# CompVis/behavior-driven-video-synthesis

Hardware: AMD Instinct MI355X
Metric: frames/sec VUnet 256x256 bs=16 fwd+bwd (higher is better)
Workload: dtype f32 (operands scaled by a power of two and split into 2 fp16 terms, 3 partial products on fp16 MFMA, fp32 accumulate; weight gradients and uncovered layers: 3 bf16 terms / 6 products, fp32-input MFMA, fp32 VALU); 1 GPU; Human3.6m shape_and_pose_net VunetAlter 256x256 per-GPU bs=16 fwd+bwd, VGG19 perceptual + KL loss, fused Adam, dropout 0.05, regressor side loop off, seeded-synthetic VGG19 weights, rasterised synthetic stickmen; global_batch=16, parallelism=dp1, conv_precision=h2, hip_streams=4, hip_graph=True, graph_settle_steps=7, rccl_world_size=1, dp_backend=none

## Files before the change

### behavior_driven_video_synthesis_amd/csrc/conv_p2.hip

```cpp
#include <stdio.h>

#include <type_traits>

#include "common.h"
#include "split_h2.h"

namespace {

constexpr int P2_META = 128, P2_AMAX0 = 16, P2_NSLOT = 64;

struct P2Args {
  const uint4* x;
  const int* xmeta;
  const uint4* w;
  const float* wk;
  const float* shift;
  const uint4* mask;
  uint4* y;
  int* ymeta;
  int N, C, H, W, M;
  int relu;
};

__device__ __forceinline__ void p2_dma(uint32_t voff, const void* sbase, uint32_t lds_addr) {
  uint32_t keep;
  asm volatile("s_mov_b32 %0, m0\n\ts_mov_b32 m0, %3\n\ts_nop 0\n\tglobal_load_lds_dwordx4 %1, %2\n\ts_mov_b32 m0, %0"
               : "=&s"(keep)
               : "v"(voff), "s"(sbase), "s"(lds_addr)
               : "memory");
}
template <int N>
__device__ __forceinline__ void p2_dma_wait() {
  static_assert(N == 0 || N == 1 || N == 2 || N == 4, "counts in use");
  if constexpr (N == 0) asm volatile("s_waitcnt vmcnt(0)" ::: "memory");
  else if constexpr (N == 1) asm volatile("s_waitcnt vmcnt(1)" ::: "memory");
  else if constexpr (N == 2) asm volatile("s_waitcnt vmcnt(2)" ::: "memory");
// ... 16 lines not shown

__device__ __forceinline__ void p2_swap16(uint32_t& a, uint32_t& b) {
  const auto r = __builtin_amdgcn_permlane16_swap(a, b, false, false);
  a = r[0];
  b = r[1];
}

__device__ __forceinline__ uint32_t p2_nonzero_halves(uint32_t t) {
  typedef unsigned short u16x2 __attribute__((ext_vector_type(2)));
  u16x2 v = __builtin_bit_cast(u16x2, t);
  const u16x2 one = {1, 1}, all = {0xFFFF, 0xFFFF};
  v = __builtin_elementwise_min(v, one) * all;
  return __builtin_bit_cast(uint32_t, v);
}

#define P2_TERMS 2
#include "conv_p2_kernel.h"
#undef P2_TERMS
#define P2_TERMS 1
#include "conv_p2_kernel.h"
#undef P2_TERMS

template <int CT, int TERMS>
int p2a_launch(const P2Args& a, hipStream_t st) {
  constexpr int XU = 4 * TERMS * 10 * (CT + 2), XS = (XU + 63) / 64 * 64, WU = 128 * 4 * TERMS;
  constexpr size_t lds = (size_t)(2 * XS + 2 * WU) * 16;
  const int blocks = a.N * (a.H / 8) * (a.W / CT) * (a.M / 128);
  void (*kern)(const P2Args);
  if constexpr (TERMS == 2) kern = conv_p2a_kernel<CT>;
  else kern = conv_p2a_kernel<CT, 1>;
  if (hipFuncSetAttribute((const void*)kern, hipFuncAttributeMaxDynamicSharedMemorySize, (int)lds) != hipSuccess) return VUNET_ERR_LAUNCH;
  VUNET_LAUNCH(kern, dim3((unsigned)blocks), dim3(512), lds, st, a);
  return vunet_check_launch();
}

template <int NW, int CT, int XBUF, int TERMS>
int p2_launch(const P2Args& a, hipStream_t st) {
  constexpr int XU = 4 * TERMS * 10 * (CT + 2), XS = (XU + 63) / 64 * 64, WU = 16 * NW * 4 * TERMS;
  constexpr size_t lds = (size_t)(XBUF * XS + 2 * WU) * 16;
  const int blocks = a.N * (a.H / 8) * (a.W / CT) * (a.M / (16 * NW));
  void (*kern)(const P2Args);
  if constexpr (TERMS == 2) kern = conv_p2_kernel<NW, CT, XBUF>;
  else kern = conv_p2_kernel<NW, CT, XBUF, 1>;
  if (lds > 64 * 1024 && hipFuncSetAttribute((const void*)kern, hipFuncAttributeMaxDynamicSharedMemorySize, (int)lds) != hipSuccess)
    return VUNET_ERR_LAUNCH;
  VUNET_LAUNCH(kern, dim3((unsigned)blocks), dim3(64 * NW), lds, st, a);
  return vunet_check_launch();
}

}

static bool p2_shape_ok(const vunet_p2_desc* d) {
  if (!d || d->N < 1 || d->C < 32 || d->C % 32 || d->M < 64 || d->M % 64 || d->H < 8 || d->H % 8) return false;
  if (!(d->W == 16 || (d->W >= 32 && d->W % 32 == 0))) return false;
  const double plane_bytes = (double)d->N * (d->C / 8) * (d->H + 2) * (d->W + 2) * 16.0;
  return plane_bytes * 2.0 < 4.0e9;
}

// ... 11 lines not shown
  int form;
  bool lockstep;
  int xbuf;
};
static P2Route p2_route(const vunet_p2_desc* d, bool dgrad) {
  const int mode = g_vunet_tune[VUNET_TUNE_P2_TERMS], force = g_vunet_tune[VUNET_TUNE_P2_FORM];
  if (mode == 3 && dgrad) {
    if (d->M % 128 == 0 && (force == 2 || force == 3)) return {1, 8, false, 2};
    const long wgs = (long)d->N * (d->H / 8) * (d->W / (d->W == 16 ? 16 : 32)) * (d->M / 64);
    return {1, 4, false, force != 1 && wgs <= 256 ? 2 : 1};
  }
  const int terms = mode == 1 ? 1 : 2, form = p2_form(d);
  return {terms, form, terms == 2 && force == 3, form == 8 ? 2 : 1};
}

extern "C" int vunet_p2_conv(const vunet_p2_desc* d, const void* x, const int32_t* xmeta, const void* w_image, const float* wk,
                             const float* shift, const void* mask, void* y, int32_t* ymeta, void* stream) {
  if (!d || !x || !xmeta || !w_image || !wk || !y || !ymeta) return VUNET_ERR_ARG;
  if (!p2_shape_ok(d)) return VUNET_ERR_UNSUPPORTED;
  if (((uintptr_t)x | (uintptr_t)w_image | (uintptr_t)y | (uintptr_t)mask | (uintptr_t)shift) & 15) return VUNET_ERR_ARG;
  P2Args a;
  a.x = (const uint4*)x; a.xmeta = xmeta; a.w = (const uint4*)w_image; a.wk = wk; a.shift = shift; a.mask = (const uint4*)mask;
  a.y = (uint4*)y; a.ymeta = ymeta;
  a.N = d->N; a.C = d->C; a.H = d->H; a.W = d->W; a.M = d->M; a.relu = d->relu;
  hipStream_t st = (hipStream_t)stream;
  const P2Route r = p2_route(d, d->relu == 0 && shift == nullptr);
  if (r.terms == 2) {
    if (d->W == 16) return r.form == 8 ? (r.lockstep ? p2_launch<8, 16, 2, 2>(a, st) : p2a_launch<16, 2>(a, st)) : p2_launch<4, 16, 1, 2>(a, st);
    return r.form == 8 ? (r.lockstep ? p2_launch<8, 32, 2, 2>(a, st) : p2a_launch<32, 2>(a, st)) : p2_launch<4, 32, 1, 2>(a, st);
  }
  if (r.form == 8 || r.xbuf == 1) {
    if (d->W == 16) return r.form == 8 ? p2a_launch<16, 1>(a, st) : p2_launch<4, 16, 1, 1>(a, st);
    return r.form == 8 ? p2a_launch<32, 1>(a, st) : p2_launch<4, 32, 1, 1>(a, st);
  }
  return d->W == 16 ? p2_launch<4, 16, 2, 1>(a, st) : p2_launch<4, 32, 2, 1>(a, st);
}

extern "C" int vunet_p2_conv_variant(const vunet_p2_desc* d, char* name, int32_t len) {
  if (!d || !name || len < 32) return VUNET_ERR_ARG;
  if (!p2_shape_ok(d)) return VUNET_ERR_UNSUPPORTED;
  const P2Route r = p2_route(d, d->relu == 0);
  const int ct = d->W == 16 ? 16 : 32;
  if (r.terms == 1) {
    if (r.form == 8) snprintf(name, (size_t)len, "conv_p2a_kernel<%d, 1>", ct);
    else snprintf(name, (size_t)len, "conv_p2_kernel<4, %d, %d, 1>", ct, r.xbuf);
    return VUNET_OK;
  }
  if (r.form == 8 && !r.lockstep) snprintf(name, (size_t)len, "conv_p2a_kernel<%d>", ct);
  else snprintf(name, (size_t)len, "conv_p2_kernel<%d, %d, %d>", r.form, ct, r.xbuf);
  return VUNET_OK;
// ... 145 lines not shown
    for (int j = 0; j < 8; ++j) {
      float f = src[j * HW];
      if (relu) f = f > 0.f ? f : 0.f;
      v[j] = f * s;
    }
    uint4 h, l;
    h2_split2(v[0], v[1], h.x, l.x);
    h2_split2(v[2], v[3], h.y, l.y);
    h2_split2(v[4], v[5], h.z, l.z);
    h2_split2(v[6], v[7], h.w, l.w);
    const size_t o = (t * Hp + (yh + 1)) * Wp + (xw + 1);
    y[o] = h;
    y[plane + o] = l;
  }
}
__device__ __forceinline__ void p2_unpack(const uint4& h, const uint4& l, float inv, float* v) {
  const uint32_t hs[4] = {h.x, h.y, h.z, h.w}, ls[4] = {l.x, l.y, l.z, l.w};
#pragma unroll
  for (int j = 0; j < 4; ++j) {
    const h2_f16x2 a = __builtin_bit_cast(h2_f16x2, hs[j]), b = __builtin_bit_cast(h2_f16x2, ls[j]);
    v[2 * j] = ((float)a[0] + (float)b[0] * (1.f / 2048.f)) * inv;
    v[2 * j + 1] = ((float)a[1] + (float)b[1] * (1.f / 2048.f)) * inv;
  }
}
__global__ __launch_bounds__(256) void p2_to_nchw_kernel(const uint4* __restrict__ x, const int* __restrict__ xmeta,
                                                         float* __restrict__ y, int N, int C, int H, int W) {
  const int CB = C >> 3, Hp = H + 2, Wp = W + 2;
  const float inv = h2_pow2(-xmeta[0]);
  const size_t HW = (size_t)H * W, total = (size_t)N * CB * HW, plane = (size_t)N * CB * Hp * Wp;
  for (size_t i = (size_t)blockIdx.x * 256 + threadIdx.x; i < total; i += (size_t)gridDim.x * 256) {
    const int xw = (int)(i % W);
    size_t t = i / W;
    const int yh = (int)(t % H);
    t /= H;
    const size_t o = (t * Hp + (yh + 1)) * Wp + (xw + 1);
    float v[8];
    p2_unpack(x[o], x[plane + o], inv, v);
    float* dst = y + (t * 8) * HW + (size_t)yh * W + xw;
#pragma unroll
// ... 27 lines not shown
```

### behavior_driven_video_synthesis_amd/csrc/conv_p2_kernel.h

```cpp
#if P2_TERMS == 2
template <int NW, int CT, int XBUF>
#else
template <int NW, int CT, int XBUF, int ONE>
#endif
__global__ __launch_bounds__(64 * NW, NW == 8 ? 1 : 2) void conv_p2_kernel(const P2Args a) {
  constexpr int TERMS = P2_TERMS;
  static_assert(NW == 4 || NW == 8, "waves");
  static_assert(CT == 32 || CT == 16, "tile width");
  static_assert(TERMS == 1 || TERMS == 2, "terms per operand");
  constexpr int MW = 16 * NW;
  constexpr int RT = 8, IH = RT + 2, CW = CT + 2, XPIX = IH * CW, XU = 4 * TERMS * XPIX;
  constexpr int NXI = (XU + 63) / 64, XS = NXI * 64;
  constexpr int NXW = (NXI + NW - 1) / NW;
  constexpr int WU = MW * 4 * TERMS;
  constexpr int NWI = WU / 64 / NW;
  constexpr int WSRC = TERMS == 2 ? 1024 : 2048;
  constexpr int PTR = CT / 16, NPT = 2 * PTR;
  static_assert(XBUF == 1 || NXW <= 8, "the next chunk's pieces ride on the first taps");
  extern __shared__ __attribute__((aligned(16))) uint4 smem[];
  uint4* const xL = smem;
  uint4* const wL = smem + XBUF * XS;

  const int tid = threadIdx.x, lane = tid & 63;
  const int wave = __builtin_amdgcn_readfirstlane(tid >> 6);
// ... 43 lines not shown
  };
  auto issue_w = [&](int g, int buf) {
    const char* src = wsrc0 + (size_t)g * wslab;
#pragma unroll
    for (int i = 0; i < NWI; ++i) {
      const int part = wave * NWI + i;
      p2_dma(lane16, p2_uniform_ptr(src + (size_t)part * WSRC), wL_addr + (uint32_t)(buf * WU + part * 64) * 16u);
    }
  };

  issue_w(0, 0);
#pragma unroll
  for (int i = 0; i < NXW; ++i) issue_x(0, i);

  float descale, descale2, sy;
  {
    const int ex = a.xmeta[0];
    const float amax_x = p2_meta_amax(a.xmeta, lane);
    const int ew = (int)a.wk[2];
    h2_pow2_pair(-(ex + ew), descale, descale2);
    const float bound = a.wk[0] * amax_x + a.wk[1];
    const int ey = h2_scale_exp(bound);
    sy = h2_pow2(ey);
    if (blockIdx.x == 0 && tid == 0) a.ymeta[0] = ey;
  }

  f32x4 acc[4][NPT], acx[4][NPT];
#pragma unroll
  for (int mt = 0; mt < 4; ++mt)
#pragma unroll
    for (int q = 0; q < NPT; ++q)
#pragma unroll
      for (int r = 0; r < 4; ++r) acc[mt][q][r] = acx[mt][q][r] = 0.f;

  p2_dma_wait<0>();
  __syncthreads();

// ... 93 lines not shown
      p2_swap16(ll[0][0], ll[1][0]);
      p2_swap16(ll[0][1], ll[1][1]);
      uint4 uh = make_uint4(hh[0][0], hh[0][1], hh[1][0], hh[1][1]);
      uint4 ul = make_uint4(ll[0][0], ll[0][1], ll[1][0], ll[1][1]);
      const int q = qp + (cg & 1);
      const int orow = row0 + 2 * rg + q / PTR, ocol = col0 + (q % PTR) * 16 + px;
      const int cb = ((m0 + 64 * mg + 16 * mt) >> 3) + (cg >> 1);
      const size_t o = (((size_t)n * MB + cb) * Hp + (orow + 1)) * Wp + (ocol + 1);
      if (a.mask) {
        const uint4 mh = a.mask[o], ml = a.mask[plane + o];
        const uint32_t k0 = p2_nonzero_halves((mh.x | ml.x) & 0x7FFF7FFFu), k1 = p2_nonzero_halves((mh.y | ml.y) & 0x7FFF7FFFu);
        const uint32_t k2 = p2_nonzero_halves((mh.z | ml.z) & 0x7FFF7FFFu), k3 = p2_nonzero_halves((mh.w | ml.w) & 0x7FFF7FFFu);
        uh.x &= k0; uh.y &= k1; uh.z &= k2; uh.w &= k3;
        ul.x &= k0; ul.y &= k1; ul.z &= k2; ul.w &= k3;
      }
      a.y[o] = uh;
      a.y[plane + o] = ul;
    }
  }
  {
    const float m_ = wave_max(ymax);
    if (lane == 0)
      atomicMax(reinterpret_cast<unsigned*>(a.ymeta) + P2_AMAX0 + ((blockIdx.x * NW + wave) & (P2_NSLOT - 1)), __float_as_uint(m_));
  }
}

#if P2_TERMS == 2
template <int CT>
#else
template <int CT, int ONE>
#endif
__global__ __launch_bounds__(512, 1) void conv_p2a_kernel(const P2Args a) {
  constexpr int TERMS = P2_TERMS;
  static_assert(TERMS == 1 || TERMS == 2, "terms per operand");
  constexpr int NW = 8, MW = 128;
  constexpr int RT = 8, IH = RT + 2, CW = CT + 2, XPIX = IH * CW, XU = 4 * TERMS * XPIX;
  constexpr int NXI = (XU + 63) / 64, XS = NXI * 64;
  constexpr int NXG = (NXI + 3) / 4;
  constexpr int XPT = 2, NXT = (NXG + XPT - 1) / XPT;
  constexpr int WU = MW * 4 * TERMS;
  constexpr int WSRC = TERMS == 2 ? 1024 : 2048;
  constexpr int PTR = CT / 16, NPT = 2 * PTR;
  static_assert(NXT <= 8, "the next chunk's pieces must be visible before its first tap");
  extern __shared__ __attribute__((aligned(16))) uint4 smem[];
  uint4* const xL = smem;
  uint4* const wL = smem + 2 * XS;

  const int tid = threadIdx.x, lane = tid & 63;
  const int wave = __builtin_amdgcn_readfirstlane(tid >> 6);
  const int mg = wave >> 2, rg = wave & 3;
  const int px = lane & 15, cg = lane >> 4;
  const int Hp = a.H + 2, Wp = a.W + 2, CB = a.C >> 3, MB = a.M >> 3;

  const unsigned bid = xcd_remap(blockIdx.x, gridDim.x);
  const int mblocks = a.M / MW;
  const int mb = bid % mblocks;
  int t = bid / mblocks;
  const int tiles_w = a.W / CT, tiles_h = a.H / RT;
  const int tx = t % tiles_w;
  t /= tiles_w;
  const int ty = t % tiles_h;
  const int n = t / tiles_h;
  const int row0 = ty * RT, col0 = tx * CT, m0 = mb * MW;

  uint32_t xoff[NXG];
#pragma unroll
  for (int i = 0; i < NXG; ++i) {
    int j = rg + 4 * i;
    if (j >= NXI) j = NXI - 1;
    int u = 64 * j + lane;
    if (u >= XU) u = XU - 1;
    const int p = u / (4 * XPIX);
    int rem = u - p * 4 * XPIX;
    const int kq = rem / XPIX;
    rem -= kq * XPIX;
    const int r = rem / CW, c = rem - r * CW;
    xoff[i] = (uint32_t)((((size_t)p * a.N * CB + kq) * Hp + (row0 + r)) * Wp + col0 + c) * 16u;
  }
  const uint32_t xL_addr = (uint32_t)(uintptr_t)(__attribute__((address_space(3))) void*)xL;
  const uint32_t wL_addr = (uint32_t)(uintptr_t)(__attribute__((address_space(3))) void*)wL;
  const char* const xsrc0 = reinterpret_cast<const char*>(a.x) + (size_t)n * CB * Hp * Wp * 16;
  const size_t xchunk = (size_t)4 * Hp * Wp * 16;
  const char* const wsrc0 = reinterpret_cast<const char*>(a.w) + (size_t)mb * (MW / 16) * 128 * 16;
  const size_t wslab = (size_t)(a.M / 16) * 128 * 16;
  const uint32_t lane16 = (uint32_t)lane * 16u;

  auto issue_x = [&](int ch, int i) {
    int j = rg + 4 * i;
    if (j >= NXI) j = NXI - 1;
    if constexpr (TERMS == 1) j = __builtin_amdgcn_readfirstlane(j);
    p2_dma(xoff[i], p2_uniform_ptr(xsrc0 + (size_t)ch * xchunk), xL_addr + (uint32_t)((ch & 1) * XS + 64 * j) * 16u);
  };
  auto issue_w = [&](int g, int buf) {
    const char* src = wsrc0 + (size_t)g * wslab;
#pragma unroll
    for (int i = 0; i < 2 * TERMS; ++i) {
      const int part = rg * (2 * TERMS) + i;
      p2_dma(lane16, p2_uniform_ptr(src + (size_t)part * WSRC), wL_addr + (uint32_t)(buf * WU + part * 64) * 16u);
    }
  };

  if (mg == 0) issue_w(0, 0);
  else {
#pragma unroll
    for (int i = 0; i < NXG; ++i) issue_x(0, i);
  }
  float descale, descale2, sy;
  {
    const int ex = a.xmeta[0];
    const float amax_x = p2_meta_amax(a.xmeta, lane);
    const int ew = (int)a.wk[2];
    h2_pow2_pair(-(ex + ew), descale, descale2);
    const float bound = a.wk[0] * amax_x + a.wk[1];
    const int ey = h2_scale_exp(bound);
    sy = h2_pow2(ey);
    if (blockIdx.x == 0 && tid == 0) a.ymeta[0] = ey;
  }
  f32x4 acc[4][NPT], acx[4][NPT];
#pragma unroll
  for (int mt = 0; mt < 4; ++mt)
#pragma unroll
    for (int q = 0; q < NPT; ++q)
#pragma unroll
      for (int r = 0; r < 4; ++r) acc[mt][q][r] = acx[mt][q][r] = 0.f;
  p2_dma_wait<0>();
  __syncthreads();
  if (mg == 1) __builtin_amdgcn_s_barrier();

  const int nch = a.C >> 5;
  const uint4* const wA0 = wL + (mg * 4) * (64 * TERMS) + lane;
  const uint4* const xB0 = xL + cg * XPIX + px + (2 * rg) * CW;

  auto chunk = [&](int ch, auto last_c) {
    constexpr bool LAST = decltype(last_c)::value;
    const uint4* const xB = xB0 + (ch & 1) * XS;
    const int wpar = (ch * 9) & 1;
#pragma unroll
    for (int tap = 0; tap < 9; ++tap) {
      const int kh = tap / 3, kw = tap - 3 * kh;
      const int g = ch * 9 + tap;
      const int buf = wpar ^ (tap & 1);
      const bool more_w = !(LAST && tap == 8);
      if (mg == 0) {
        if (more_w) issue_w(g + 1, buf ^ 1);
      } else if (!LAST && tap < NXT) {
#pragma unroll
        for (int i = 0; i < XPT; ++i)
          if (tap * XPT + i < NXG) issue_x(ch + 1, tap * XPT + i);
      }
      const uint4* const wA = wA0 + buf * WU;
      P2Unit av[TERMS][4], bv[TERMS][NPT];
#pragma unroll
      for (int p = 0; p < TERMS; ++p) {
#pragma unroll
        for (int mt = 0; mt < 4; ++mt) av[p][mt].u = wA[(mt * TERMS + p) * 64];
#pragma unroll
        for (int q = 0; q < NPT; ++q) bv[p][q].u = xB[p * 4 * XPIX + (q / PTR + kh) * CW + (q % PTR) * 16 + kw];
      }
      asm volatile("s_waitcnt lgkmcnt(0)" ::: "memory");
      __builtin_amdgcn_sched_barrier(0);
      __builtin_amdgcn_s_barrier();
      __builtin_amdgcn_sched_barrier(0);
      __builtin_amdgcn_s_setprio(1);
// ... 9 lines not shown
          for (int q = 0; q < NPT; ++q)
            acx[mt][q] = __builtin_amdgcn_mfma_f32_16x16x32_f16(av[0][mt].b, bv[TERMS - 1][q].b, acx[mt][q], 0, 0, 0);
      }
#pragma unroll
      for (int mt = 0; mt < 4; ++mt)
#pragma unroll
        for (int q = 0; q < NPT; ++q)
          acc[mt][q] = __builtin_amdgcn_mfma_f32_16x16x32_f16(av[0][mt].b, bv[0][q].b, acc[mt][q], 0, 0, 0);
      __builtin_amdgcn_s_setprio(0);
      __builtin_amdgcn_sched_barrier(0);
      p2_dma_wait<0>();
      __builtin_amdgcn_s_barrier();
      __builtin_amdgcn_sched_barrier(0);
    }
  };
  for (int ch = 0; ch + 1 < nch; ++ch) chunk(ch, std::false_type{});
  chunk(nch - 1, std::true_type{});
  if (mg == 0) __builtin_amdgcn_s_barrier();

  const bool relu = a.relu != 0;
  const size_t plane = (size_t)a.N * MB * Hp * Wp;
  float ymax = 0.f;
#pragma unroll
  for (int mt = 0; mt < 4; ++mt) {
    const int co = m0 + 64 * mg + 16 * mt + 4 * cg;
    float sh[4] = {0.f, 0.f, 0.f, 0.f};
    if (a.shift) {
      const float4 s4 = *reinterpret_cast<const float4*>(a.shift + co);
      sh[0] = s4.x; sh[1] = s4.y; sh[2] = s4.z; sh[3] = s4.w;
    }
#pragma unroll
    for (int qp = 0; qp < NPT; qp += 2) {
      uint32_t hh[2][2], ll[2][2];
#pragma unroll
      for (int s = 0; s < 2; ++s) {
        float v[4];
#pragma unroll
        for (int r = 0; r < 4; ++r) {
          float c;
          if constexpr (TERMS == 2) c = (acc[mt][qp + s][r] + acx[mt][qp + s][r] * (1.f / 2048.f)) * descale * descale2 + sh[r];
          else c = acc[mt][qp + s][r] * descale * descale2 + sh[r];
          c = (relu && !(c > 0.f)) ? 0.f : c;
          ymax = fmaxf(ymax, fabsf(c));
          v[r] = c * sy;
        }
        h2_split2(v[0], v[1], hh[s][0], ll[s][0]);
        h2_split2(v[2], v[3], hh[s][1], ll[s][1]);
      }
      p2_swap16(hh[0][0], hh[1][0]);
      p2_swap16(hh[0][1], hh[1][1]);
      p2_swap16(ll[0][0], ll[1][0]);
      p2_swap16(ll[0][1], ll[1][1]);
      uint4 uh = make_uint4(hh[0][0], hh[0][1], hh[1][0], hh[1][1]);
      uint4 ul = make_uint4(ll[0][0], ll[0][1], ll[1][0], ll[1][1]);
      const int q = qp + (cg & 1);
      const int orow = row0 + 2 * rg + q / PTR, ocol = col0 + (q % PTR) * 16 + px;
      const int cb = ((m0 + 64 * mg + 16 * mt) >> 3) + (cg >> 1);
      const size_t o = (((size_t)n * MB + cb) * Hp + (orow + 1)) * Wp + (ocol + 1);
      if (a.mask) {
        const uint4 mh = a.mask[o], ml = a.mask[plane + o];
        const uint32_t k0 = p2_nonzero_halves((mh.x | ml.x) & 0x7FFF7FFFu), k1 = p2_nonzero_halves((mh.y | ml.y) & 0x7FFF7FFFu);
        const uint32_t k2 = p2_nonzero_halves((mh.z | ml.z) & 0x7FFF7FFFu), k3 = p2_nonzero_halves((mh.w | ml.w) & 0x7FFF7FFFu);
        uh.x &= k0; uh.y &= k1; uh.z &= k2; uh.w &= k3;
        ul.x &= k0; ul.y &= k1; ul.z &= k2; ul.w &= k3;
      }
      a.y[o] = uh;
      a.y[plane + o] = ul;
    }
  }
  {
    const float m_ = wave_max(ymax);
    if (lane == 0)
      atomicMax(reinterpret_cast<unsigned*>(a.ymeta) + P2_AMAX0 + ((blockIdx.x * NW + wave) & (P2_NSLOT - 1)), __float_as_uint(m_));
  }
}
```

### behavior_driven_video_synthesis_amd/models/imagenet_pretrained.py

```python
from __future__ import annotations

import math

import torch
from torch import nn

from .. import ops
from ..lib.modules import Conv2d

VGG19_CFG = [64, 64, "M", 128, 128, "M", 256, 256, 256, 256, "M", 512, 512, 512, 512, "M", 512, 512, 512, 512, "M"]


class _Marker(nn.Module):

    def __init__(self, kind):
        super().__init__()
        self.kind = kind


class VGG19(nn.Module):

    def __init__(self, width_div: int = 1):
        super().__init__()
        layers, cin = [], 3
# ... 203 lines not shown
    def forward(self, role, xp, targets=None, tap_weights=None):
        st = self._role(role)
        st["metas"].zero_()
        A = st["A"]
        _, wt_f, _, shift, _, wk = self._first()
        n, _, h, w = xp.shape
        amax = ops._tagged_amax(xp)
        if amax is None:
            amax = ops.absmax_partials(xp)
        ops._call("vunet_p2_conv_first", ops._p(xp), ops._p(amax), 512, ops._p(wt_f), int(wt_f.shape[1]), ops._p(shift), ops._p(wk),
                  ops._p(A[0].buf), ops._p(A[0].meta), n, h, w, A[0].shape[1], ops._stream())
        taps, losses = {}, {}
        steps = self.program[1]
        for k, step in enumerate(steps, start=1):
            if step[0] == "conv":
                ops.p2_conv(A[k - 1], self._weights(step[1]), A[k], relu=True)
                tap = step[2]
                if tap is not None:
                    taps[tap] = A[k]
                    pool_next = k < len(steps) and steps[k][0] == "pool"
                    if targets is not None and not pool_next:
                        losses[tap] = ops.p2_l1_fwd(targets[tap], A[k], tap_weights[tap])
            else:
                prev = steps[k - 2] if k >= 2 else None
                tap = prev[2] if (prev is not None and prev[0] == "conv") else None
                if targets is not None and tap is not None:
                    losses[tap] = ops.p2_pool_fwd(A[k - 1], A[k], t=targets[tap], weight=tap_weights[tap])
                else:
                    ops.p2_pool_fwd(A[k - 1], A[k])
        return taps, losses

    def backward(self, targets, tap_weights, gouts):
        st = self.roles["p"]
        A, steps = st["A"], self.program[1]
        L = len(steps)

        def tap_scale(tap, k):
            c, h, w = st["shp"][k]
            return float(tap_weights[tap]) / (self.geo[0] * c * h * w)

        def has(tap):
            return tap is not None and gouts.get(tap) is not None
        k = L
        top = steps[L - 1][2]
        D = None
        if has(top):
            D = ops.p2_l1_bwd(targets[top], A[L], None, self._grad_buf(st, "G", L), tap_scale(top, L), gouts[top])
        while k >= 1:
            step = steps[k - 1]
            if step[0] == "pool":
                prev = steps[k - 2]
                tap = prev[2] if has(prev[2]) else None
                if D is None and tap is None:
                    k -= 1
                    continue
                if D is None:
                    D = ops.p2_l1_bwd(targets[tap], A[k - 1], None, self._grad_buf(st, "G", k - 1), tap_scale(tap, k - 1), gouts[tap])
                else:
                    D = ops.p2_pool_bwd(A[k - 1], D, self._grad_buf(st, "G", k - 1), t=None if tap is None else targets[tap],
                                        gscale=0.0 if tap is None else tap_scale(tap, k - 1), gout=None if tap is None else gouts[tap])
                k -= 1
                continue
            below = steps[k - 2] if k >= 2 else None
            if D is None:
                tap = below[2] if (below is not None and below[0] == "conv" and has(below[2])) else None
                if tap is not None:
                    D = ops.p2_l1_bwd(targets[tap], A[k - 1], None, self._grad_buf(st, "G", k - 1), tap_scale(tap, k - 1), gouts[tap])
                k -= 1
                continue
            wts = self._weights(step[1])
            if below is None:
                D = ops.p2_conv(D, wts, self._grad_buf(st, "G", 0), dgrad=True, mask=A[0])
            elif below[0] == "pool":
                D = ops.p2_conv(D, wts, self._grad_buf(st, "G", k - 1), dgrad=True)
            elif has(below[2]):
                up = ops.p2_conv(D, wts, self._grad_buf(st, "U", k - 1), dgrad=True)
                D = ops.p2_l1_bwd(targets[below[2]], A[k - 1], up, self._grad_buf(st, "G", k - 1), tap_scale(below[2], k - 1),
                                  gouts[below[2]])
            else:
                D = ops.p2_conv(D, wts, self._grad_buf(st, "G", k - 1), dgrad=True, mask=A[k - 1])
            k -= 1
        if D is None:
            return None
        _, _, wt_d, _, wx_d, _ = self._first()
        n, h, w = self.geo
        c0 = st["shp"][0][0]
        dconv = D.to_nchw()
        dx = torch.empty(n, 3, h, w, device=self.device, dtype=torch.float32)
        ops._conv_gather(ops._dgrad_desc(n, c0, h, w, 3, h, w, 3, 1, 1, wt_d.shape[1]), dconv, None, wt_d, None, None, None, dx, wx_d)
        return dx


class P2VggLoss(torch.autograd.Function):

    @staticmethod
    def forward(ctx, xp, engine, target, tap_weights, names):
        _, losses = engine.forward("p", xp, target.planes, tap_weights)
        engine.pred_generation += 1
        ctx.engine, ctx.target, ctx.tap_weights, ctx.names = engine, target, tap_weights, names
        ctx.generation, ctx.pred_generation = target.generation, engine.pred_generation
        return tuple(losses[n] for n in names)

# ... 132 lines not shown
```

### behavior_driven_video_synthesis_amd/ops.py

```python
from __future__ import annotations

import contextlib
import ctypes
import os
from collections import namedtuple
from dataclasses import dataclass
from typing import Optional, Tuple

import torch

from . import _lib

ACT_NONE, ACT_ELU, ACT_RELU, ACT_SIGMOID, ACT_LRELU = 0, 1, 2, 3, 4
SEED2_OFFSET = 0x9E3779B9


class ConvDesc(ctypes.Structure):
    _fields_ = [("N", ctypes.c_int32), ("C1", ctypes.c_int32), ("C2", ctypes.c_int32), ("Hs", ctypes.c_int32),
                ("Ws", ctypes.c_int32), ("M", ctypes.c_int32), ("m_off", ctypes.c_int32), ("Mpad", ctypes.c_int32),
                ("Ho", ctypes.c_int32), ("Wo", ctypes.c_int32), ("KH", ctypes.c_int32), ("KW", ctypes.c_int32),
                ("stride", ctypes.c_int32), ("pad", ctypes.c_int32), ("mode", ctypes.c_int32),
                ("in_act", ctypes.c_int32), ("in_slope", ctypes.c_float), ("drop_p", ctypes.c_float),
                ("drop_seed", ctypes.c_uint32), ("out_act", ctypes.c_int32), ("d2s", ctypes.c_int32),
                ("aux_act", ctypes.c_int32), ("aux_slope", ctypes.c_float), ("aux_drop_p", ctypes.c_float),
# ... 1720 lines not shown
                  self.cout, self.cin, int(dgrad), _p(img), _p(wk), _p(work), _stream())
            rec = self._img[dgrad] = (stamp, img, wk)
        return rec[1], rec[2]


def p2_conv_supported(n, c, h, w, m) -> bool:
    d = P2Desc(n, c, h, w, m, 0)
    return _lib.lib().vunet_p2_conv_supported(ctypes.byref(d)) == 1


def _p2_key(d, dgrad):
    return (("conv_gather_dgrad" if dgrad else "conv_gather_fwd", d.N, d.C, 0, d.H, d.W, d.M, 3, 1, 0,
             _kernel_name("vunet_p2_conv_variant", ctypes.byref(d))), 2.0 * d.N * d.H * d.W * d.C * d.M * 9)


def p2_conv(x: Planes, wts: P2Weights, out: Planes, relu: bool = True, dgrad: bool = False, mask: Planes = None):
    n, c, h, w = x.shape
    m = wts.cin if dgrad else wts.cout
    assert c == (wts.cout if dgrad else wts.cin) and out.shape == (n, m, h, w)
    img, wk = wts.image(dgrad)
    d = P2Desc(n, c, h, w, m, int(relu and not dgrad))
    with _timed(_p2_key, d, dgrad):
        _call("vunet_p2_conv", ctypes.byref(d), _p(x.buf), _p(x.meta), _p(img), _p(wk),
              _p(None if dgrad or wts.bias is None else wts.bias), _p(None if mask is None else mask.buf), _p(out.buf), _p(out.meta),
              _stream())
    return out


def p2_l1_fwd(t: Planes, p: Planes, weight: float):
    n, c, h, w = p.shape
    assert t.shape == p.shape
    out = _zero_scalar(p.buf.device)
    partial = torch.empty(1024, device=p.buf.device, dtype=torch.float32)
    _call("vunet_p2_l1_fwd", _p(t.buf), _p(t.meta), _p(p.buf), _p(p.meta), _p(partial), _p(out), float(weight), n, c, h, w, _stream())
    return out


def p2_pool_fwd(p: Planes, out: Planes, t: Planes = None, weight: float = 0.0):
    n, c, h, w = p.shape
    assert out.shape == (n, c, h // 2, w // 2)
    loss = partial = None
# ... 21 lines not shown
```

### include/vunet_hip.h

```cpp
#ifndef VUNET_HIP_H
#define VUNET_HIP_H
#include <stddef.h>
#include <stdint.h>

#ifdef __cplusplus
extern "C" {
#endif

#define VUNET_OK 0
#define VUNET_ERR_ARG (-1)
#define VUNET_ERR_LAUNCH (-2)
#define VUNET_ERR_UNSUPPORTED (-3)

#define VUNET_ACT_NONE 0
#define VUNET_ACT_ELU 1
#define VUNET_ACT_RELU 2
#define VUNET_ACT_SIGMOID 3
#define VUNET_ACT_LRELU 4

int vunet_abi_version(void);

typedef struct vunet_conv_desc {
  int32_t N;
  int32_t C1, C2;
// ... 235 lines not shown
int vunet_unit_sample(const float* mu, const float* logstd, float* z, float* eps_out, int64_t n, uint32_t seed, void* stream);

int vunet_set_schedule(double* lr_dev, double lr, float* imax_dev, float imax, int32_t* step_dev, int32_t step, void* stream);

int vunet_sum_amax(const float* const* srcs, int32_t n, float* out, float* amax_out, int64_t numel, void* stream);

typedef struct vunet_p2_desc {
  int32_t N, C, H, W;
  int32_t M;
  int32_t relu;
} vunet_p2_desc;
int vunet_p2_conv_supported(const vunet_p2_desc* d);
int vunet_p2_conv_variant(const vunet_p2_desc* d, char* name, int32_t len);
int vunet_p2_conv(const vunet_p2_desc* d, const void* x, const int32_t* xmeta, const void* w_image, const float* wk,
                  const float* shift, const void* mask, void* y, int32_t* ymeta, void* stream);
int vunet_p2_weight_image_bytes(int32_t Cout, int32_t Cin, int32_t dgrad);
int vunet_p2_pack_weights(const float* w, const float* shift, int32_t Cout, int32_t Cin, int32_t dgrad, void* image, float* wk,
                          float* workspace, void* stream);
int vunet_p2_weight_bound(const float* w, const float* shift, int32_t Cout, int32_t Cin, float* wk, float* workspace, void* stream);
int vunet_p2_conv_first(const float* x, const float* amax_x, int32_t n_amax, const float* wt_f, int32_t Mpad, const float* shift,
                        const float* wk, void* y, int32_t* ymeta, int32_t N, int32_t H, int32_t W, int32_t M, void* stream);
int vunet_p2_from_nchw(const float* x, const float* amax, int32_t n_amax, int32_t relu, void* y, int32_t* ymeta, int32_t N,
                       int32_t C, int32_t H, int32_t W, void* stream);
int vunet_p2_to_nchw(const void* x, const int32_t* xmeta, float* y, int32_t N, int32_t C, int32_t H, int32_t W, void* stream);

int vunet_p2_l1_fwd(const void* t, const int32_t* tmeta, const void* p, const int32_t* pmeta, float* partial, float* out,
                    float weight, int32_t N, int32_t C, int32_t H, int32_t W, void* stream);
int vunet_p2_pool_fwd(const void* t, const int32_t* tmeta, const void* p, const int32_t* pmeta, float* partial, float* out,
                      float weight, void* y, int32_t* ymeta, int32_t N, int32_t C, int32_t H, int32_t W, void* stream);
int vunet_p2_l1_bwd(const void* t, const int32_t* tmeta, const void* p, const int32_t* pmeta, const void* add,
// ... 47 lines not shown
```

Baseline: 794.2 frames/s.

## Make p2a conv persistent with cross-tile prefetch; fuse fp32 NCHW epilogue into dgrad

The 8-wave p2a conv kernel becomes persistent: the grid is capped at the CU count and each workgroup loops over tiles, prefetching the next tile's weights and activations during the last chunk of the current tile so the DMA pipeline stays busy across tile boundaries. Mask loads are hoisted ahead of the epilogue, and the loop-invariant scale factors are made scalar-uniform. A new fp32 NCHW-output variant of the 4-wave kernel lets the first-layer VGG dgrad write NCHW floats directly, removing the separate to_nchw conversion pass. Target-branch VGG forward convs opt out of persistence, and a fixed grid cap can leave CUs idle or unbalanced when the tile count is not a multiple of it.

```diff
diff --git a/behavior_driven_video_synthesis_amd/csrc/conv_p2.hip b/behavior_driven_video_synthesis_amd/csrc/conv_p2.hip
--- a/behavior_driven_video_synthesis_amd/csrc/conv_p2.hip
+++ b/behavior_driven_video_synthesis_amd/csrc/conv_p2.hip
@@ -20,6 +20,7 @@
   int* ymeta;
   int N, C, H, W, M;
   int relu;
+  float* y32;
 };
 
 __device__ __forceinline__ void p2_dma(uint32_t voff, const void* sbase, uint32_t lds_addr) {
@@ -66,18 +67,52 @@
   return __builtin_bit_cast(uint32_t, v);
 }
 
+__device__ __forceinline__ void p2_unpack(const uint4& h, const uint4& l, float inv, float* v) {
+  const uint32_t hs[4] = {h.x, h.y, h.z, h.w}, ls[4] = {l.x, l.y, l.z, l.w};
+#pragma unroll
+  for (int j = 0; j < 4; ++j) {
+    const h2_f16x2 a = __builtin_bit_cast(h2_f16x2, hs[j]), b = __builtin_bit_cast(h2_f16x2, ls[j]);
+    v[2 * j] = ((float)a[0] + (float)b[0] * (1.f / 2048.f)) * inv;
+    v[2 * j + 1] = ((float)a[1] + (float)b[1] * (1.f / 2048.f)) * inv;
+  }
+}
+
 #define P2_TERMS 2
 #include "conv_p2_kernel.h"
 #undef P2_TERMS
 #define P2_TERMS 1
 #include "conv_p2_kernel.h"
 #undef P2_TERMS
+#undef P2_F32OUT
+#define P2_F32OUT 1
+#define P2_TERMS 2
+#include "conv_p2_kernel.h"
+#undef P2_TERMS
+#define P2_TERMS 1
+#include "conv_p2_kernel.h"
+#undef P2_TERMS
+#undef P2_F32OUT
+
+int g_p2_wg_limit = 0;
+int p2_wg_limit() {
+  if (g_p2_wg_limit > 0) return g_p2_wg_limit;
+  static int cus[64];
+  int dev = 0;
+  if (hipGetDevice(&dev) != hipSuccess || dev < 0 || dev >= 64) return 1 << 30;
+  if (cus[dev] == 0) {
+    int n = 0;
+    if (hipDeviceGetAttribute(&n, hipDeviceAttributeMultiprocessorCount, dev) != hipSuccess || n < 1) return 1 << 30;
+    cus[dev] = n;
+  }
+  return cus[dev];
+}
 
 template <int CT, int TERMS>
 int p2a_launch(const P2Args& a, hipStream_t st) {
   constexpr int XU = 4 * TERMS * 10 * (CT + 2), XS = (XU + 63) / 64 * 64, WU = 128 * 4 * TERMS;
   constexpr size_t lds = (size_t)(2 * XS + 2 * WU) * 16;
-  const int blocks = a.N * (a.H / 8) * (a.W / CT) * (a.M / 128);
+  const int tiles = a.N * (a.H / 8) * (a.W / CT) * (a.M / 128), limit = p2_wg_limit();
+  const int blocks = tiles < limit ? tiles : limit;
   void (*kern)(const P2Args);
   if constexpr (TERMS == 2) kern = conv_p2a_kernel<CT>;
   else kern = conv_p2a_kernel<CT, 1>;
@@ -94,6 +129,12 @@
   void (*kern)(const P2Args);
   if constexpr (TERMS == 2) kern = conv_p2_kernel<NW, CT, XBUF>;
   else kern = conv_p2_kernel<NW, CT, XBUF, 1>;
+  if constexpr (NW == 4) {
+    if (a.y32) {
+      if constexpr (TERMS == 2) kern = conv_p2_nchw_kernel<NW, CT, XBUF>;
+      else kern = conv_p2_nchw_kernel<NW, CT, XBUF, 1>;
+    }
+  }
   if (lds > 64 * 1024 && hipFuncSetAttribute((const void*)kern, hipFuncAttributeMaxDynamicSharedMemorySize, (int)lds) != hipSuccess)
     return VUNET_ERR_LAUNCH;
   VUNET_LAUNCH(kern, dim3((unsigned)blocks), dim3(64 * NW), lds, st, a);
@@ -135,17 +176,18 @@
   return {terms, form, terms == 2 && force == 3, form == 8 ? 2 : 1};
 }
 
-extern "C" int vunet_p2_conv(const vunet_p2_desc* d, const void* x, const int32_t* xmeta, const void* w_image, const float* wk,
-                             const float* shift, const void* mask, void* y, int32_t* ymeta, void* stream) {
-  if (!d || !x || !xmeta || !w_image || !wk || !y || !ymeta) return VUNET_ERR_ARG;
+static int p2_conv_run(const vunet_p2_desc* d, const void* x, const int32_t* xmeta, const void* w_image, const float* wk,
+                       const float* shift, const void* mask, void* y, float* y32, int32_t* ymeta, void* stream) {
+  if (!d || !x || !xmeta || !w_image || !wk || (!y && !y32) || !ymeta) return VUNET_ERR_ARG;
   if (!p2_shape_ok(d)) return VUNET_ERR_UNSUPPORTED;
-  if (((uintptr_t)x | (uintptr_t)w_image | (uintptr_t)y | (uintptr_t)mask | (uintptr_t)shift) & 15) return VUNET_ERR_ARG;
+  if (((uintptr_t)x | (uintptr_t)w_image | (uintptr_t)y | (uintptr_t)y32 | (uintptr_t)mask | (uintptr_t)shift) & 15) return VUNET_ERR_ARG;
   P2Args a;
   a.x = (const uint4*)x; a.xmeta = xmeta; a.w = (const uint4*)w_image; a.wk = wk; a.shift = shift; a.mask = (const uint4*)mask;
-  a.y = (uint4*)y; a.ymeta = ymeta;
+  a.y = (uint4*)y; a.ymeta = ymeta; a.y32 = y32;
   a.N = d->N; a.C = d->C; a.H = d->H; a.W = d->W; a.M = d->M; a.relu = d->relu;
   hipStream_t st = (hipStream_t)stream;
   const P2Route r = p2_route(d, d->relu == 0 && shift == nullptr);
+  if (y32 && r.form != 4) return VUNET_ERR_UNSUPPORTED;
   if (r.terms == 2) {
     if (d->W == 16) return r.form == 8 ? (r.lockstep ? p2_launch<8, 16, 2, 2>(a, st) : p2a_launch<16, 2>(a, st)) : p2_launch<4, 16, 1, 2>(a, st);
     return r.form == 8 ? (r.lockstep ? p2_launch<8, 32, 2, 2>(a, st) : p2a_launch<32, 2>(a, st)) : p2_launch<4, 32, 1, 2>(a, st);
@@ -155,6 +197,24 @@
     return r.form == 8 ? p2a_launch<32, 1>(a, st) : p2_launch<4, 32, 1, 1>(a, st);
   }
   return d->W == 16 ? p2_launch<4, 16, 2, 1>(a, st) : p2_launch<4, 32, 2, 1>(a, st);
+}
+
+extern "C" int vunet_p2_conv(const vunet_p2_desc* d, const void* x, const int32_t* xmeta, const void* w_image, const float* wk,
+                             const float* shift, const void* mask, void* y, int32_t* ymeta, void* stream) {
+  if (!y) return VUNET_ERR_ARG;
+  return p2_conv_run(d, x, xmeta, w_image, wk, shift, mask, y, nullptr, ymeta, stream);
+}
+
+extern "C" int vunet_p2_conv_nchw(const vunet_p2_desc* d, const void* x, const int32_t* xmeta, const void* w_image, const float* wk,
+                                  const float* shift, const void* mask, float* y, int32_t* ymeta, void* stream) {
+  if (!y) return VUNET_ERR_ARG;
+  return p2_conv_run(d, x, xmeta, w_image, wk, shift, mask, nullptr, y, ymeta, stream);
+}
+
+extern "C" int vunet_p2_set_wg_limit(int32_t limit) {
+  if (limit < 0) return VUNET_ERR_ARG;
+  g_p2_wg_limit = limit;
+  return VUNET_OK;
 }
 
 extern "C" int vunet_p2_conv_variant(const vunet_p2_desc* d, char* name, int32_t len) {
@@ -330,15 +390,6 @@
     y[plane + o] = l;
   }
 }
-__device__ __forceinline__ void p2_unpack(const uint4& h, const uint4& l, float inv, float* v) {
-  const uint32_t hs[4] = {h.x, h.y, h.z, h.w}, ls[4] = {l.x, l.y, l.z, l.w};
-#pragma unroll
-  for (int j = 0; j < 4; ++j) {
-    const h2_f16x2 a = __builtin_bit_cast(h2_f16x2, hs[j]), b = __builtin_bit_cast(h2_f16x2, ls[j]);
-    v[2 * j] = ((float)a[0] + (float)b[0] * (1.f / 2048.f)) * inv;
-    v[2 * j + 1] = ((float)a[1] + (float)b[1] * (1.f / 2048.f)) * inv;
-  }
-}
 __global__ __launch_bounds__(256) void p2_to_nchw_kernel(const uint4* __restrict__ x, const int* __restrict__ xmeta,
                                                          float* __restrict__ y, int N, int C, int H, int W) {
   const int CB = C >> 3, Hp = H + 2, Wp = W + 2;
diff --git a/behavior_driven_video_synthesis_amd/csrc/conv_p2_kernel.h b/behavior_driven_video_synthesis_amd/csrc/conv_p2_kernel.h
--- a/behavior_driven_video_synthesis_amd/csrc/conv_p2_kernel.h
+++ b/behavior_driven_video_synthesis_amd/csrc/conv_p2_kernel.h
@@ -1,10 +1,20 @@
+#ifndef P2_F32OUT
+#define P2_F32OUT 0
+#endif
+#if P2_F32OUT
+#define P2_KERNEL conv_p2_nchw_kernel
+#else
+#define P2_KERNEL conv_p2_kernel
+#endif
 #if P2_TERMS == 2
 template <int NW, int CT, int XBUF>
 #else
 template <int NW, int CT, int XBUF, int ONE>
 #endif
-__global__ __launch_bounds__(64 * NW, NW == 8 ? 1 : 2) void conv_p2_kernel(const P2Args a) {
+__global__ __launch_bounds__(64 * NW, NW == 8 ? 1 : 2) void P2_KERNEL(const P2Args a) {
   constexpr int TERMS = P2_TERMS;
+  constexpr bool F32OUT = P2_F32OUT != 0;
+  static_assert(!F32OUT || NW == 4, "the fp32 epilogue: four-wave forms");
   static_assert(NW == 4 || NW == 8, "waves");
   static_assert(CT == 32 || CT == 16, "tile width");
   static_assert(TERMS == 1 || TERMS == 2, "terms per operand");
@@ -81,13 +91,14 @@
   for (int i = 0; i < NXW; ++i) issue_x(0, i);
 
   float descale, descale2, sy;
+  int ey;
   {
     const int ex = a.xmeta[0];
     const float amax_x = p2_meta_amax(a.xmeta, lane);
     const int ew = (int)a.wk[2];
     h2_pow2_pair(-(ex + ew), descale, descale2);
     const float bound = a.wk[0] * amax_x + a.wk[1];
-    const int ey = h2_scale_exp(bound);
+    ey = h2_scale_exp(bound);
     sy = h2_pow2(ey);
     if (blockIdx.x == 0 && tid == 0) a.ymeta[0] = ey;
   }
@@ -211,8 +222,17 @@
         uh.x &= k0; uh.y &= k1; uh.z &= k2; uh.w &= k3;
         ul.x &= k0; ul.y &= k1; ul.z &= k2; ul.w &= k3;
       }
-      a.y[o] = uh;
-      a.y[plane + o] = ul;
+      if constexpr (F32OUT) {
+        float v8[8];
+        p2_unpack(uh, ul, h2_pow2(-ey), v8);
+        const size_t HW = (size_t)a.H * a.W;
+        float* const dst = a.y32 + ((size_t)n * a.M + 8 * cb) * HW + (size_t)orow * a.W + ocol;
+#pragma unroll
+        for (int j = 0; j < 8; ++j) dst[j * HW] = v8[j];
+      } else {
+        a.y[o] = uh;
+        a.y[plane + o] = ul;
+      }
     }
   }
   {
@@ -222,6 +242,8 @@
   }
 }
 
+#undef P2_KERNEL
+#if !P2_F32OUT
 #if P2_TERMS == 2
 template <int CT>
 #else
@@ -249,16 +271,32 @@
   const int px = lane & 15, cg = lane >> 4;
   const int Hp = a.H + 2, Wp = a.W + 2, CB = a.C >> 3, MB = a.M >> 3;
 
-  const unsigned bid = xcd_remap(blockIdx.x, gridDim.x);
   const int mblocks = a.M / MW;
-  const int mb = bid % mblocks;
-  int t = bid / mblocks;
   const int tiles_w = a.W / CT, tiles_h = a.H / RT;
-  const int tx = t % tiles_w;
-  t /= tiles_w;
-  const int ty = t % tiles_h;
-  const int n = t / tiles_h;
-  const int row0 = ty * RT, col0 = tx * CT, m0 = mb * MW;
+  const int ntiles = a.N * tiles_h * tiles_w * mblocks;
+  const int G = (int)gridDim.x;
+  struct Tile {
+    const char* xsrc;
+    const char* wsrc;
+    size_t y0;
+    int m0;
+  };
+  auto tile_at = [&](int t) {
+    Tile g;
+    const int mb = t % mblocks;
+    t /= mblocks;
+    const int tx = t % tiles_w;
+    t /= tiles_w;
+    const int ty = t % tiles_h;
+    const int n = t / tiles_h, row0 = ty * RT, col0 = tx * CT;
+    g.m0 = mb * MW;
+    g.xsrc = reinterpret_cast<const char*>(a.x) + ((size_t)n * CB * Hp * Wp + (size_t)row0 * Wp + col0) * 16;
+    g.wsrc = reinterpret_cast<const char*>(a.w) + (size_t)mb * (MW / 16) * 128 * 16;
+    g.y0 = (((size_t)n * MB + (g.m0 >> 3)) * Hp + (row0 + 1)) * Wp + (col0 + 1);
+    return g;
+  };
+  int tile = (int)xcd_remap(blockIdx.x, gridDim.x);
+  Tile cur = tile_at(tile), nxt = cur;
 
   uint32_t xoff[NXG];
 #pragma unroll
@@ -272,24 +310,21 @@
     const int kq = rem / XPIX;
     rem -= kq * XPIX;
     const int r = rem / CW, c = rem - r * CW;
-    xoff[i] = (uint32_t)((((size_t)p * a.N * CB + kq) * Hp + (row0 + r)) * Wp + col0 + c) * 16u;
+    xoff[i] = (uint32_t)((((size_t)p * a.N * CB + kq) * Hp + r) * Wp + c) * 16u;
   }
   const uint32_t xL_addr = (uint32_t)(uintptr_t)(__attribute__((address_space(3))) void*)xL;
   const uint32_t wL_addr = (uint32_t)(uintptr_t)(__attribute__((address_space(3))) void*)wL;
-  const char* const xsrc0 = reinterpret_cast<const char*>(a.x) + (size_t)n * CB * Hp * Wp * 16;
   const size_t xchunk = (size_t)4 * Hp * Wp * 16;
-  const char* const wsrc0 = reinterpret_cast<const char*>(a.w) + (size_t)mb * (MW / 16) * 128 * 16;
   const size_t wslab = (size_t)(a.M / 16) * 128 * 16;
   const uint32_t lane16 = (uint32_t)lane * 16u;
 
-  auto issue_x = [&](int ch, int i) {
+  auto issue_x = [&](const char* src, int xb, int i) {
     int j = rg + 4 * i;
     if (j >= NXI) j = NXI - 1;
     if constexpr (TERMS == 1) j = __builtin_amdgcn_readfirstlane(j);
-    p2_dma(xoff[i], p2_uniform_ptr(xsrc0 + (size_t)ch * xchunk), xL_addr + (uint32_t)((ch & 1) * XS + 64 * j) * 16u);
-  };
-  auto issue_w = [&](int g, int buf) {
-    const char* src = wsrc0 + (size_t)g * wslab;
+    p2_dma(xoff[i], p2_uniform_ptr(src), xL_addr + (uint32_t)(xb * XS + 64 * j) * 16u);
+  };
+  auto issue_w = [&](const char* src, int buf) {
 #pragma unroll
     for (int i = 0; i < 2 * TERMS; ++i) {
       const int part = rg * (2 * TERMS) + i;
@@ -297,10 +332,10 @@
     }
   };
 
-  if (mg == 0) issue_w(0, 0);
+  if (mg == 0) issue_w(cur.wsrc, 0);
   else {
 #pragma unroll
-    for (int i = 0; i < NXG; ++i) issue_x(0, i);
+    for (int i = 0; i < NXG; ++i) issue_x(cur.xsrc, 0, i);
   }
   float descale, descale2, sy;
   {
@@ -312,14 +347,23 @@
     const int ey = h2_scale_exp(bound);
     sy = h2_pow2(ey);
     if (blockIdx.x == 0 && tid == 0) a.ymeta[0] = ey;
+    descale = __int_as_float(__builtin_amdgcn_readfirstlane(__float_as_int(descale)));
+    descale2 = __int_as_float(__builtin_amdgcn_readfirstlane(__float_as_int(descale2)));
+    sy = __int_as_float(__builtin_amdgcn_readfirstlane(__float_as_int(sy)));
   }
   f32x4 acc[4][NPT], acx[4][NPT];
-#pragma unroll
-  for (int mt = 0; mt < 4; ++mt)
-#pragma unroll
-    for (int q = 0; q < NPT; ++q)
-#pragma unroll
-      for (int r = 0; r < 4; ++r) acc[mt][q][r] = acx[mt][q][r] = 0.f;
+  auto zero_acc = [&]() {
+#pragma unroll
+    for (int mt = 0; mt < 4; ++mt)
+#pragma unroll
+      for (int q = 0; q < NPT; ++q)
+#pragma unroll
+        for (int r = 0; r < 4; ++r) {
+          asm volatile("v_mov_b32 %0, 0" : "+v"(acc[mt][q][r]));
+          if constexpr (TERMS == 2) asm volatile("v_mov_b32 %0, 0" : "+v"(acx[mt][q][r]));
+        }
+  };
+  zero_acc();
   p2_dma_wait<0>();
   __syncthreads();
   if (mg == 1) __builtin_amdgcn_s_barrier();
@@ -328,22 +372,18 @@
   const uint4* const wA0 = wL + (mg * 4) * (64 * TERMS) + lane;
   const uint4* const xB0 = xL + cg * XPIX + px + (2 * rg) * CW;
 
-  auto chunk = [&](int ch, auto last_c) {
-    constexpr bool LAST = decltype(last_c)::value;
-    const uint4* const xB = xB0 + (ch & 1) * XS;
-    const int wpar = (ch * 9) & 1;
+  auto chunk = [&](int par, const char* wsrc, const char* wnext, const char* xnext, bool has_next) {
+    const uint4* const xB = xB0 + par * XS;
 #pragma unroll
     for (int tap = 0; tap < 9; ++tap) {
       const int kh = tap / 3, kw = tap - 3 * kh;
-      const int g = ch * 9 + tap;
-      const int buf = wpar ^ (tap & 1);
-      const bool more_w = !(LAST && tap == 8);
+      const int buf = par ^ (tap & 1);
       if (mg == 0) {
-        if (more_w) issue_w(g + 1, buf ^ 1);
-      } else if (!LAST && tap < NXT) {
+        if (tap < 8 || has_next) issue_w(tap == 8 ? wnext : wsrc + (size_t)(tap + 1) * wslab, buf ^ 1);
+      } else if (tap < NXT && has_next) {
 #pragma unroll
         for (int i = 0; i < XPT; ++i)
-          if (tap * XPT + i < NXG) issue_x(ch + 1, tap * XPT + i);
+          if (tap * XPT + i < NXG) issue_x(xnext, par ^ 1, tap * XPT + i);
       }
       const uint4* const wA = wA0 + buf * WU;
       P2Unit av[TERMS][4], bv[TERMS][NPT];
@@ -383,59 +423,95 @@
       __builtin_amdgcn_sched_barrier(0);
     }
   };
-  for (int ch = 0; ch + 1 < nch; ++ch) chunk(ch, std::false_type{});
-  chunk(nch - 1, std::true_type{});
-  if (mg == 0) __builtin_amdgcn_s_barrier();
-
   const bool relu = a.relu != 0;
   const size_t plane = (size_t)a.N * MB * Hp * Wp;
   float ymax = 0.f;
-#pragma unroll
-  for (int mt = 0; mt < 4; ++mt) {
-    const int co = m0 + 64 * mg + 16 * mt + 4 * cg;
-    float sh[4] = {0.f, 0.f, 0.f, 0.f};
-    if (a.shift) {
-      const float4 s4 = *reinterpret_cast<const float4*>(a.shift + co);
-      sh[0] = s4.x; sh[1] = s4.y; sh[2] = s4.z; sh[3] = s4.w;
-    }
-#pragma unroll
-    for (int qp = 0; qp < NPT; qp += 2) {
-      uint32_t hh[2][2], ll[2][2];
-#pragma unroll
-      for (int s = 0; s < 2; ++s) {
-        float v[4];
-#pragma unroll
-        for (int r = 0; r < 4; ++r) {
-          float c;
-          if constexpr (TERMS == 2) c = (acc[mt][qp + s][r] + acx[mt][qp + s][r] * (1.f / 2048.f)) * descale * descale2 + sh[r];
-          else c = acc[mt][qp + s][r] * descale * descale2 + sh[r];
-          c = (relu && !(c > 0.f)) ? 0.f : c;
-          ymax = fmaxf(ymax, fabsf(c));
-          v[r] = c * sy;
+
+  auto epilogue = [&](const Tile& g) {
+    const int m0 = g.m0;
+    int lane_e = lane;
+    asm volatile("" : "+v"(lane_e));
+    const int px = lane_e & 15, cg = lane_e >> 4;
+    auto unit_off = [&](int mt, int qp) {
+      const int q = qp + (cg & 1);
+      const int orow = 2 * rg + q / PTR, ocol = (q % PTR) * 16 + px;
+      const int cb = ((64 * mg + 16 * mt) >> 3) + (cg >> 1);
+      return g.y0 + ((size_t)cb * Hp + orow) * Wp + ocol;
+    };
+    uint4 mkh[4][NPT / 2], mkl[4][NPT / 2];
+    if (a.mask) {
+#pragma unroll
+      for (int mt = 0; mt < 4; ++mt)
+#pragma unroll
+        for (int qp = 0; qp < NPT; qp += 2) {
+          const size_t o = unit_off(mt, qp);
+          mkh[mt][qp / 2] = a.mask[o];
+          mkl[mt][qp / 2] = a.mask[plane + o];
         }
-        h2_split2(v[0], v[1], hh[s][0], ll[s][0]);
-        h2_split2(v[2], v[3], hh[s][1], ll[s][1]);
-      }
-      p2_swap16(hh[0][0], hh[1][0]);
-      p2_swap16(hh[0][1], hh[1][1]);
-      p2_swap16(ll[0][0], ll[1][0]);
-      p2_swap16(ll[0][1], ll[1][1]);
-      uint4 uh = make_uint4(hh[0][0], hh[0][1], hh[1][0], hh[1][1]);
-      uint4 ul = make_uint4(ll[0][0], ll[0][1], ll[1][0], ll[1][1]);
-      const int q = qp + (cg & 1);
-      const int orow = row0 + 2 * rg + q / PTR, ocol = col0 + (q % PTR) * 16 + px;
-      const int cb = ((m0 + 64 * mg + 16 * mt) >> 3) + (cg >> 1);
-      const size_t o = (((size_t)n * MB + cb) * Hp + (orow + 1)) * Wp + (ocol + 1);
-      if (a.mask) {
-        const uint4 mh = a.mask[o], ml = a.mask[plane + o];
-        const uint32_t k0 = p2_nonzero_halves((mh.x | ml.x) & 0x7FFF7FFFu), k1 = p2_nonzero_halves((mh.y | ml.y) & 0x7FFF7FFFu);
-        const uint32_t k2 = p2_nonzero_halves((mh.z | ml.z) & 0x7FFF7FFFu), k3 = p2_nonzero_halves((mh.w | ml.w) & 0x7FFF7FFFu);
-        uh.x &= k0; uh.y &= k1; uh.z &= k2; uh.w &= k3;
-        ul.x &= k0; ul.y &= k1; ul.z &= k2; ul.w &= k3;
-      }
-      a.y[o] = uh;
-      a.y[plane + o] = ul;
-    }
+    }
+#pragma unroll
+    for (int mt = 0; mt < 4; ++mt) {
+      const int co = m0 + 64 * mg + 16 * mt + 4 * cg;
+      float sh[4] = {0.f, 0.f, 0.f, 0.f};
+      if (a.shift) {
+        const float4 s4 = *reinterpret_cast<const float4*>(a.shift + co);
+        sh[0] = s4.x; sh[1] = s4.y; sh[2] = s4.z; sh[3] = s4.w;
+      }
+#pragma unroll
+      for (int qp = 0; qp < NPT; qp += 2) {
+        uint32_t hh[2][2], ll[2][2];
+#pragma unroll
+        for (int s = 0; s < 2; ++s) {
+          float v[4];
+#pragma unroll
+          for (int r = 0; r < 4; ++r) {
+            float c;
+            if constexpr (TERMS == 2) c = (acc[mt][qp + s][r] + acx[mt][qp + s][r] * (1.f / 2048.f)) * descale * descale2 + sh[r];
+            else c = acc[mt][qp + s][r] * descale * descale2 + sh[r];
+            c = (relu && !(c > 0.f)) ? 0.f : c;
+            ymax = fmaxf(ymax, fabsf(c));
+            v[r] = c * sy;
+          }
+          h2_split2(v[0], v[1], hh[s][0], ll[s][0]);
+          h2_split2(v[2], v[3], hh[s][1], ll[s][1]);
+        }
+        p2_swap16(hh[0][0], hh[1][0]);
+        p2_swap16(hh[0][1], hh[1][1]);
+        p2_swap16(ll[0][0], ll[1][0]);
+        p2_swap16(ll[0][1], ll[1][1]);
+        uint4 uh = make_uint4(hh[0][0], hh[0][1], hh[1][0], hh[1][1]);
+        uint4 ul = make_uint4(ll[0][0], ll[0][1], ll[1][0], ll[1][1]);
+        const size_t o = unit_off(mt, qp);
+        if (a.mask) {
+          const uint4 mh = mkh[mt][qp / 2], ml = mkl[mt][qp / 2];
+          const uint32_t k0 = p2_nonzero_halves((mh.x | ml.x) & 0x7FFF7FFFu), k1 = p2_nonzero_halves((mh.y | ml.y) & 0x7FFF7FFFu);
+          const uint32_t k2 = p2_nonzero_halves((mh.z | ml.z) & 0x7FFF7FFFu), k3 = p2_nonzero_halves((mh.w | ml.w) & 0x7FFF7FFFu);
+          uh.x &= k0; uh.y &= k1; uh.z &= k2; uh.w &= k3;
+          ul.x &= k0; ul.y &= k1; ul.z &= k2; ul.w &= k3;
+        }
+        a.y[o] = uh;
+        a.y[plane + o] = ul;
+      }
+    }
+  };
+
+  int par = 0;
+  for (;;) {
+    const bool more_tiles = tile + G < ntiles;
+    for (int ch = 0; ch < nch; ++ch) {
+      const bool tile_end = ch + 1 == nch;
+      const char* const wsrc = cur.wsrc + (size_t)(ch * 9) * wslab;
+      if (tile_end && more_tiles) nxt = tile_at(tile + G);
+      chunk(par, wsrc, tile_end ? nxt.wsrc : wsrc + (size_t)9 * wslab, tile_end ? nxt.xsrc : cur.xsrc + (size_t)(ch + 1) * xchunk,
+            !tile_end || more_tiles);
+      par ^= 1;
+    }
+    if (!more_tiles && mg == 0) __builtin_amdgcn_s_barrier();
+    epilogue(cur);
+    if (!more_tiles) break;
+    cur = nxt;
+    tile += G;
+    zero_acc();
   }
   {
     const float m_ = wave_max(ymax);
@@ -443,3 +519,4 @@
       atomicMax(reinterpret_cast<unsigned*>(a.ymeta) + P2_AMAX0 + ((blockIdx.x * NW + wave) & (P2_NSLOT - 1)), __float_as_uint(m_));
   }
 }
+#endif
diff --git a/behavior_driven_video_synthesis_amd/models/imagenet_pretrained.py b/behavior_driven_video_synthesis_amd/models/imagenet_pretrained.py
--- a/behavior_driven_video_synthesis_amd/models/imagenet_pretrained.py
+++ b/behavior_driven_video_synthesis_amd/models/imagenet_pretrained.py
@@ -241,7 +241,7 @@
         steps = self.program[1]
         for k, step in enumerate(steps, start=1):
             if step[0] == "conv":
-                ops.p2_conv(A[k - 1], self._weights(step[1]), A[k], relu=True)
+                ops.p2_conv(A[k - 1], self._weights(step[1]), A[k], relu=True, persistent=role != "t")
                 tap = step[2]
                 if tap is not None:
                     taps[tap] = A[k]
@@ -271,6 +271,7 @@
         k = L
         top = steps[L - 1][2]
         D = None
+        dconv = None
         if has(top):
             D = ops.p2_l1_bwd(targets[top], A[L], None, self._grad_buf(st, "G", L), tap_scale(top, L), gouts[top])
         while k >= 1:
@@ -297,7 +298,9 @@
                 continue
             wts = self._weights(step[1])
             if below is None:
-                D = ops.p2_conv(D, wts, self._grad_buf(st, "G", 0), dgrad=True, mask=A[0])
+                g0 = self._grad_buf(st, "G", 0)
+                dconv = torch.empty(g0.shape, device=self.device, dtype=torch.float32)
+                D = ops.p2_conv(D, wts, g0, dgrad=True, mask=A[0], out_nchw=dconv)
             elif below[0] == "pool":
                 D = ops.p2_conv(D, wts, self._grad_buf(st, "G", k - 1), dgrad=True)
             elif has(below[2]):
@@ -312,7 +315,8 @@
         _, _, wt_d, _, wx_d, _ = self._first()
         n, h, w = self.geo
         c0 = st["shp"][0][0]
-        dconv = D.to_nchw()
+        if dconv is None:
+            dconv = D.to_nchw()
         dx = torch.empty(n, 3, h, w, device=self.device, dtype=torch.float32)
         ops._conv_gather(ops._dgrad_desc(n, c0, h, w, 3, h, w, 3, 1, 1, wt_d.shape[1]), dconv, None, wt_d, None, None, None, dx, wx_d)
         return dx
diff --git a/behavior_driven_video_synthesis_amd/ops.py b/behavior_driven_video_synthesis_amd/ops.py
--- a/behavior_driven_video_synthesis_amd/ops.py
+++ b/behavior_driven_video_synthesis_amd/ops.py
@@ -1758,17 +1758,48 @@
              _kernel_name("vunet_p2_conv_variant", ctypes.byref(d))), 2.0 * d.N * d.H * d.W * d.C * d.M * 9)
 
 
-def p2_conv(x: Planes, wts: P2Weights, out: Planes, relu: bool = True, dgrad: bool = False, mask: Planes = None):
+def _p2_key_nchw(d, dgrad):
+    key, flop = _p2_key(d, dgrad)
+    return key[:-1] + (key[-1].replace("conv_p2_kernel<", "conv_p2_nchw_kernel<"),), flop
+
+
+_P2_ONE_TILE_PER_WG = 1 << 30
+_p2_wg_limit = 0
+
+
+def p2_conv(x: Planes, wts: P2Weights, out: Planes, relu: bool = True, dgrad: bool = False, mask: Planes = None, out_nchw=None,
+            persistent: bool = True):
+    if not persistent:
+        _call("vunet_p2_set_wg_limit", _P2_ONE_TILE_PER_WG)
+        try:
+            return p2_conv(x, wts, out, relu=relu, dgrad=dgrad, mask=mask, out_nchw=out_nchw)
+        finally:
+            _call("vunet_p2_set_wg_limit", _p2_wg_limit)
     n, c, h, w = x.shape
     m = wts.cin if dgrad else wts.cout
     assert c == (wts.cout if dgrad else wts.cin) and out.shape == (n, m, h, w)
     img, wk = wts.image(dgrad)
     d = P2Desc(n, c, h, w, m, int(relu and not dgrad))
+    shift = _p(None if dgrad or wts.bias is None else wts.bias)
+    if out_nchw is not None:
+        _dev(out_nchw)
+        if not (out_nchw.dtype == torch.float32 and out_nchw.is_contiguous() and tuple(out_nchw.shape) == (n, m, h, w)):
+            raise RuntimeError("p2_conv: out_nchw must be a contiguous fp32 [N, M, H, W] tensor")
+        with _timed(_p2_key_nchw, d, dgrad):
+            _call("vunet_p2_conv_nchw", ctypes.byref(d), _p(x.buf), _p(x.meta), _p(img), _p(wk), shift,
+                  _p(None if mask is None else mask.buf), _p(out_nchw), _p(out.meta), _stream())
+        return out_nchw
     with _timed(_p2_key, d, dgrad):
         _call("vunet_p2_conv", ctypes.byref(d), _p(x.buf), _p(x.meta), _p(img), _p(wk),
-              _p(None if dgrad or wts.bias is None else wts.bias), _p(None if mask is None else mask.buf), _p(out.buf), _p(out.meta),
+              shift, _p(None if mask is None else mask.buf), _p(out.buf), _p(out.meta),
               _stream())
     return out
+
+
+def set_p2_wg_limit(limit: int = 0) -> None:
+    global _p2_wg_limit
+    _call("vunet_p2_set_wg_limit", int(limit))
+    _p2_wg_limit = int(limit)
 
 
 def p2_l1_fwd(t: Planes, p: Planes, weight: float):
diff --git a/include/vunet_hip.h b/include/vunet_hip.h
--- a/include/vunet_hip.h
+++ b/include/vunet_hip.h
@@ -273,6 +273,9 @@
 int vunet_p2_conv_variant(const vunet_p2_desc* d, char* name, int32_t len);
 int vunet_p2_conv(const vunet_p2_desc* d, const void* x, const int32_t* xmeta, const void* w_image, const float* wk,
                   const float* shift, const void* mask, void* y, int32_t* ymeta, void* stream);
+int vunet_p2_conv_nchw(const vunet_p2_desc* d, const void* x, const int32_t* xmeta, const void* w_image, const float* wk,
+                       const float* shift, const void* mask, float* y, int32_t* ymeta, void* stream);
+int vunet_p2_set_wg_limit(int32_t limit);
 int vunet_p2_weight_image_bytes(int32_t Cout, int32_t Cin, int32_t dgrad);
 int vunet_p2_pack_weights(const float* w, const float* shift, int32_t Cout, int32_t Cin, int32_t dgrad, void* image, float* wk,
                           float* workspace, void* stream);
```

Result: no change. 797.5 frames/s (median of 2 runs) (+0.4%).
